# ADicksonLab/AGDIFF

Hardware: AMD Instinct MI355X
Metric: conformers/sec (whole node), GEOM-Drugs 5000-step sampling (higher is better)
Workload: dtype f16x3

## Files before the change

### agdiff_amd/csrc/common.hpp

```cpp
#pragma once
#include <hip/hip_runtime.h>
#include <stdint.h>
#include "agdiff_hip.h"

typedef float f32x4 __attribute__((ext_vector_type(4)));
typedef __bf16 bf16x8 __attribute__((ext_vector_type(8)));
typedef _Float16 f16x8 __attribute__((ext_vector_type(8)));
typedef unsigned int u32x4 __attribute__((ext_vector_type(4)));
typedef __attribute__((address_space(3))) u32x4 lds_u32x4;

#define AG_WAVE 64
#define AG_WG 256
#define AG_TW AGDIFF_TILE

__device__ __forceinline__ int ag_lane() { return threadIdx.x & 63; }
__device__ __forceinline__ int ag_wave_in_wg() { return threadIdx.x >> 6; }

__device__ __forceinline__ f32x4 ag_ld4(const float* __restrict__ p) { return *reinterpret_cast<const f32x4*>(p); }
__device__ __forceinline__ void ag_st4(float* __restrict__ p, f32x4 v) { *reinterpret_cast<f32x4*>(p) = v; }

__device__ __forceinline__ float ag_exp2(float x) { return __builtin_amdgcn_exp2f(x); }
__device__ __forceinline__ float ag_log2(float x) { return __builtin_amdgcn_logf(x); }
__device__ __forceinline__ float ag_rcp(float x) { return __builtin_amdgcn_rcpf(x); }

// ... 238 lines not shown
  } else {
    using V = decltype(x.hi);
    const V wv = __builtin_bit_cast(V, w[part == 2 ? 1 : 0]);
    const V xv = (part == 1) ? x.lo : x.hi;
    o = FLIP ? ag_mfma16(xv, wv, o) : ag_mfma16(wv, xv, o);
  }
}

template <int MODE, bool FLIP>
__device__ __forceinline__ void ag_block_mma_mixed(f32x4& o, const AgIn<MODE>& x, const u32x4 (&w)[2]) {
  static_assert(MODE != AG_F32, "split modes only");
  using V = decltype(x.hi);
  const V wv = __builtin_bit_cast(V, w[1]);
  o = FLIP ? ag_mfma16(x.lo, wv, o) : ag_mfma16(wv, x.lo, o);
}

template <int MODE, bool FLIP>
__device__ __forceinline__ f32x4 ag_block_mma_first(const AgIn<MODE>& x, const u32x4 (&w)[2]) {
  const f32x4 zero = {0.f, 0.f, 0.f, 0.f};
  if constexpr (MODE == AG_F32) {
    const f32x4 wf = __builtin_bit_cast(f32x4, w[0]);
    return FLIP ? __builtin_amdgcn_mfma_f32_16x16x4f32(x.v[0][0], wf[0], zero, 0, 0, 0)
                : __builtin_amdgcn_mfma_f32_16x16x4f32(wf[0], x.v[0][0], zero, 0, 0, 0);
  } else {
    using V = decltype(x.hi);
    const V wv = __builtin_bit_cast(V, w[0]);
    return FLIP ? ag_mfma16(x.hi, wv, zero) : ag_mfma16(wv, x.hi, zero);
  }
}

template <int MODE, bool FLIP, bool KOUTER, int KT, int OT, int X0, int O0, int PF, int NX, int NO>
__device__ __forceinline__ void ag_dense(const AgIn<MODE> (&x)[NX], f32x4 (&o)[NO], const void* wpk, int lane) {
  static_assert(X0 + KT <= NX && O0 + OT <= NO, "tile range");
  constexpr int S = OT * KT;
  constexpr int R = PF + 1;
  u32x4 w[R][2];
  const u32x4* wl = reinterpret_cast<const u32x4*>(wpk) + lane;
#pragma unroll
  for (int s = 0; s < (PF < S ? PF : S); ++s) {
    w[s % R][0] = wl[(s * 2) * 64];
    w[s % R][1] = wl[(s * 2 + 1) * 64];
  }
#pragma unroll
  for (int s = 0; s < S; ++s) {
    const int t = KOUTER ? s / OT : s % KT, ot = KOUTER ? s % OT : s / KT;
    if (s + PF < S) {
      w[(s + PF) % R][0] = wl[((s + PF) * 2) * 64];
      w[(s + PF) % R][1] = wl[((s + PF) * 2 + 1) * 64];
    }
    ag_block_mma<MODE, FLIP>(o[O0 + ot], x[X0 + t], w[s % R]);
    __builtin_amdgcn_sched_barrier(0);
  }
}
template <int MODE, bool FLIP, bool KOUTER, int KT, int OT, int X0, int O0, int NX, int NO>
__device__ __forceinline__ void ag_dense_lds(const AgIn<MODE> (&x)[NX], f32x4 (&o)[NO], const lds_u32x4* wl, int lane) {
  static_assert(X0 + KT <= NX && O0 + OT <= NO, "tile range");
  constexpr int G = (OT % 4 == 0) ? 4 : (OT % 2 == 0) ? 2 : 1;
#pragma unroll
  for (int og = 0; og < OT / G; ++og) {
#pragma unroll
    for (int t = 0; t < KT; ++t) {
      u32x4 w[G][2];
#pragma unroll
      for (int g = 0; g < G; ++g) {
        const int ot = og * G + g;
        const int s = KOUTER ? t * OT + ot : ot * KT + t;
        w[g][0] = wl[(s * 2) * 64 + lane];
        w[g][1] = wl[(s * 2 + 1) * 64 + lane];
      }
#pragma unroll
      for (int part = 0; part < AgParts<MODE>::n; ++part) {
#pragma unroll
        for (int g = 0; g < G; ++g) ag_block_mma_part<MODE, FLIP>(o[O0 + og * G + g], x[X0 + t], w[g], part);
      }
    }
  }
}
template <int MODE, bool FLIP, bool KOUTER, int KT, int OT, int X0, int O0, int PF, int NX, int NO>
__device__ __forceinline__ void ag_dense_split(const AgIn<MODE> (&x)[NX], f32x4 (&o)[NO], const lds_u32x4* w0,
                                               const void* wpk, int lane, int lds_lane) {
  static_assert(X0 + KT <= NX && O0 + OT <= NO, "tile range");
  constexpr int S = OT * KT;
  constexpr int R = PF + 1;
  u32x4 w1[R];
  const u32x4* wl = reinterpret_cast<const u32x4*>(wpk) + 64 + lane;
#pragma unroll
  for (int s = 0; s < (PF < S ? PF : S); ++s) w1[s % R] = wl[(s * 2) * 64];
#pragma unroll
  for (int s = 0; s < S; ++s) {
    const int t = KOUTER ? s / OT : s % KT, ot = KOUTER ? s % OT : s / KT;
    if (s + PF < S) w1[(s + PF) % R] = wl[((s + PF) * 2) * 64];
    u32x4 w[2];
    w[0] = w0[s * 64 + lds_lane];
    w[1] = w1[s % R];
    ag_block_mma<MODE, FLIP>(o[O0 + ot], x[X0 + t], w);
    __builtin_amdgcn_sched_barrier(0);
  }
}
template <int MODE> struct AgPF { static constexpr int v = (MODE == AG_F32) ? 2 : 4; };
__device__ __forceinline__ const void* ag_wblock(const float* wpk, int b) { return wpk + (size_t)b * 512; }


__device__ __forceinline__ int64_t ag_attr_unit(int64_t tile, int t, int u, int lane) {
  return ((tile * 4 + t) * 2 + u) * 64 + (lane & 15) * 4 + (lane >> 4);
}
__device__ __forceinline__ void ag_store_attr(const AgIn<AG_F32>& x, float* frag, int64_t tile, int t, int lane) {
  u32x4* p = reinterpret_cast<u32x4*>(frag);
  p[ag_attr_unit(tile, t, 0, lane)] = __builtin_bit_cast(u32x4, x.v[0]);
  p[ag_attr_unit(tile, t, 1, lane)] = __builtin_bit_cast(u32x4, x.v[1]);
}
__device__ __forceinline__ void ag_store_attr(const AgIn<AG_BF3>& x, float* frag, int64_t tile, int t, int lane) {
  u32x4* p = reinterpret_cast<u32x4*>(frag);
  p[ag_attr_unit(tile, t, 0, lane)] = __builtin_bit_cast(u32x4, x.hi);
  p[ag_attr_unit(tile, t, 1, lane)] = __builtin_bit_cast(u32x4, x.lo);
}
__device__ __forceinline__ void ag_store_attr(const AgIn<AG_H3>& x, float* frag, int64_t tile, int t, int lane) {
  u32x4* p = reinterpret_cast<u32x4*>(frag);
  p[ag_attr_unit(tile, t, 0, lane)] = __builtin_bit_cast(u32x4, x.hi);
  p[ag_attr_unit(tile, t, 1, lane)] = __builtin_bit_cast(u32x4, x.lo);
}
__device__ __forceinline__ void ag_load_attr(AgIn<AG_H3>& x, const float* frag, int64_t tile, int t, int lane) {
  const u32x4* p = reinterpret_cast<const u32x4*>(frag);
  x.hi = __builtin_bit_cast(f16x8, p[ag_attr_unit(tile, t, 0, lane)]);
  x.lo = __builtin_bit_cast(f16x8, p[ag_attr_unit(tile, t, 1, lane)]);
}
__device__ __forceinline__ void ag_load_attr(AgIn<AG_F32>& x, const float* frag, int64_t tile, int t, int lane) {
  const u32x4* p = reinterpret_cast<const u32x4*>(frag);
  x.v[0] = __builtin_bit_cast(f32x4, p[ag_attr_unit(tile, t, 0, lane)]);
// ... 181 lines not shown
```

### agdiff_amd/csrc/edge.hip

```cpp
#include "common.hpp"

namespace {

__device__ __forceinline__ const lds_u32x4* ag_lds_base(const lds_u32x4* p, int lane) {
  const lds_u32x4* b = p + lane;
  asm volatile("" : "+v"(b));
  return b;
}

struct EncArgs {
  const float* fe_w;
  const float* fe_b;
  const float* t1;
  const float* w1_pk;
  const float* t3;
  const float* w23_pk;
  const float* w4_pk;
  const float* b4;
  const int32_t* n_dev;
  const float* e_len;
  const int32_t* e_type;
  float* out_frag;
  float* out_rows;
  const int32_t* row_index;
// ... 33 lines not shown
      for (int t = 0; t < 4; ++t) ag_store_attr(x[t], out_frag, tile, t, lane);
    } else {
#pragma unroll
      for (int t = 0; t < 4; ++t) {
        if (o.p >= 0) ag_store_attr(x[t], out_frag, o.p >> 4, t, q * 16 + (int)(o.p & 15));
        if (o.pm >= 0) ag_store_attr(x[t], out_frag, o.pm >> 4, t, q * 16 + (int)(o.pm & 15));
      }
    }
  }
}

#define AG_PERSIST_WAVES 16
template <int MODE>
__global__ void __launch_bounds__(64 * AG_PERSIST_WAVES, 4) k_edge_encoder(EncArgs a) {
  extern __shared__ u32x4 ag_enc_smem[];
  lds_u32x4* lw1 = (lds_u32x4*)ag_enc_smem;
  lds_u32x4* lw23 = lw1 + 32 * 128;
  lds_u32x4* lw4 = lw23 + 32 * 128;
  if (a.tile_flags && a.tile_flags[0] == 0) return;
  {
    const u32x4* g1 = reinterpret_cast<const u32x4*>(a.w1_pk);
    const u32x4* g2 = reinterpret_cast<const u32x4*>(a.w23_pk);
    const u32x4* g4 = reinterpret_cast<const u32x4*>(a.w4_pk);
    ag_copy_lds(lw1, g1, 32 * 128);
    ag_copy_lds(lw23, g2, 32 * 128);
    ag_copy_lds_map(lw4, g4, 32 * 64, [](int i) { return (i >> 6) * 128 + (i & 63); });
  }
  __syncthreads();
  const int lane0 = ag_lane();
  const int E = *a.n_dev;
  const int64_t stride = (int64_t)gridDim.x * AG_PERSIST_WAVES;
  for (int64_t tile = (int64_t)blockIdx.x * AG_PERSIST_WAVES + (threadIdx.x >> 6); tile < a.max_tiles; tile += stride) {
    if (tile * AG_TW >= E) break;
    const int row_mask = a.tile_flags ? a.tile_flags[1 + tile] : 0xFFFF;
    if (row_mask == 0) continue;
    int lane = lane0;
    asm volatile("" : "+v"(lane));
    const int q = lane >> 4;
    const int64_t e = tile * AG_TW + (lane & 15);
    const bool valid = e < E && ((row_mask >> (lane & 15)) & 1);
    const float d = valid ? a.e_len[e] : 0.0f;
    const int ty = valid ? a.e_type[e] : 0;

    f32x4 y[8];
    AgIn<MODE> x[4];
    {
      f32x4 w[8];
      ag_init_vec<8>(w, a.fe_w, q);
      ag_init_vec<8>(y, a.fe_b, q);
      AG_FOR_TILE(y, 8, ag_gelu(fmaf(w[_t][_r], d, v)));
    }
    ag_cvt_tiles<MODE, 4, 0>(y, x);
    ag_init_vec<8>(y, a.t1 + (size_t)ty * 128, q);
    ag_dense_lds<MODE, false, false, 4, 8, 0, 0>(x, y, ag_lds_base(lw1, lane), 0);
    AG_FOR_TILE(y, 8, ag_gelu(v));
    ag_cvt_tiles<MODE, 4, 0>(y, x);
    ag_init_vec<8>(y, a.t3 + (size_t)ty * 128, q);
    ag_dense_lds<MODE, false, false, 4, 8, 0, 0>(x, y, ag_lds_base(lw23, lane), 0);
    AG_FOR_TILE(y, 8, ag_gelu(v));
    ag_cvt_tiles<MODE, 4, 0>(y, x);
    ag_init_vec<8>(y, a.b4, q);
    ag_dense_split<MODE, false, false, 4, 8, 0, 0, 6>(x, y, ag_lds_base(lw4, lane), a.w4_pk, lane, 0);
    ag_emit_edge_attr<MODE>(y, ag_edge_out(a.pos_index, a.mir_index, e, valid), a.out_frag, a.out_rows, a.row_index,
                            a.pos_index != nullptr, tile, lane);
  }
}

struct GaussArgs {
  const float* offset;
  const float* emb;
  const int32_t* n_dev;
  const float* e_len;
  const int32_t* e_type;
  float* out_frag;
  float* out_rows;
  const int32_t* row_index;
  const int32_t* pos_index;
  const int32_t* mir_index;
  int64_t max_tiles;
  float coeff_log2e;
};

template <int MODE>
__global__ void __launch_bounds__(256) k_edge_gaussian(GaussArgs a) {
  const int64_t tile = (int64_t)blockIdx.x * 4 + (threadIdx.x >> 6);
  const int E = *a.n_dev;
  if (tile >= a.max_tiles || tile * AG_TW >= E) return;
  const int lane = ag_lane();
  const int q = lane >> 4;
  const int64_t e = tile * AG_TW + (lane & 15);
  const bool valid = e < E;
  const float d = valid ? a.e_len[e] : 0.0f;
  const int ty = valid ? a.e_type[e] : 0;
  f32x4 y[8];
  ag_load_row<4, 0>(y, a.offset, q);
  AG_FOR_TILE(y, 4, ag_exp2(a.coeff_log2e * ((d - v) * (d - v))));
  ag_load_row<4, 4>(y, a.emb + (size_t)ty * 64, q);
  ag_emit_edge_attr<MODE>(y, ag_edge_out(a.pos_index, a.mir_index, e, valid), a.out_frag, a.out_rows, a.row_index,
                          a.pos_index != nullptr, tile, lane);
}

struct ScaleArgs {
  const float* dw[2 * AGDIFF_MAX_CONVS];
  const int32_t* n_dev;
  const float* e_len;
  const int32_t* pos_index;
  const int32_t* mir_index;
  const int32_t* e_type;
  const int32_t* type_slot;
  float* out;
  int64_t epad;
// ... 358 lines not shown
  int64_t max_tiles;
};

template <int MODE>
__global__ void __launch_bounds__(64 * AG_PERSIST_WAVES, 4) k_pair_head(HeadArgs a) {
  extern __shared__ u32x4 ag_head_smem[];
  lds_u32x4* lw1 = (lds_u32x4*)ag_head_smem;
  lds_u32x4* lw2 = lw1 + 64 * 128;
  {
    const u32x4* g1 = reinterpret_cast<const u32x4*>(a.hp.w1_pk);
    const u32x4* g2 = reinterpret_cast<const u32x4*>(a.hp.w2_pk);
    ag_copy_lds(lw1, g1, 64 * 128);
    ag_copy_lds(lw2, g2, 16 * 128);
  }
  __syncthreads();
  const int lane0 = ag_lane();
  const int E = *a.n_dev;
  const int64_t stride = (int64_t)gridDim.x * AG_PERSIST_WAVES;
  const int64_t wg = (gridDim.x % 8 == 0) ? (int64_t)(blockIdx.x % 8) * (gridDim.x / 8) + blockIdx.x / 8 : (int64_t)blockIdx.x;
  for (int64_t tile = wg * AG_PERSIST_WAVES + (threadIdx.x >> 6); tile < a.max_tiles; tile += stride) {
    if (tile * AG_TW >= E) break;
    int lane = lane0;
    asm volatile("" : "+v"(lane));
    const int q = lane >> 4;
    const int64_t e = tile * AG_TW + (lane & 15);
    const bool valid = e < E;
    const int s = valid ? a.src[e] : 0, t = valid ? a.dst[e] : 0;
    const int64_t pe = a.pos_index ? (valid ? (int64_t)a.pos_index[e] : 0) : e;
    const int64_t pm = (a.pos_index && valid) ? (int64_t)a.mir_index[e] : -1;

    f32x4 y1[8];
    ag_init_vec<8>(y1, a.hp.b1, q);
    {
      const float* hs = a.node_h + (size_t)s * 128;
      const float* ht = a.node_h + (size_t)t * 128;
      AgIn<MODE> sl[2];
      auto load_slice = [&](AgIn<MODE>& dst, int k) {
        if (k < 4) {
          const f32x4 p0 = ag_ld4(hs + 32 * k + 4 * q) * ag_ld4(ht + 32 * k + 4 * q);
          const f32x4 p1 = ag_ld4(hs + 32 * k + 16 + 4 * q) * ag_ld4(ht + 32 * k + 16 + 4 * q);
          ag_cvt(p0, p1, dst);
        } else if (a.attr_frag && a.pos_index) {
          ag_load_attr(dst, a.attr_frag, pe >> 4, k - 4, q * 16 + (int)(pe & 15));
        } else if (a.attr_frag) {
          ag_load_attr(dst, a.attr_frag, tile, k - 4, lane);
        } else {
          const float* ar = a.attr_rows + (size_t)(valid ? e : 0) * 128 + 32 * (k - 4) + 4 * q;
          ag_cvt(ag_ld4(ar), ag_ld4(ar + 16), dst);
        }
      };
      load_slice(sl[0], 0);
      const lds_u32x4* lw1_lo = ag_lds_base(lw1, lane);
      const lds_u32x4* lw1_hi = ag_lds_base(lw1 + 32 * 128, lane);
#pragma unroll
      for (int k = 0; k < 8; ++k) {
        if (k + 1 < 8) load_slice(sl[(k + 1) & 1], k + 1);
        const lds_u32x4* wk = (k < 4) ? lw1_lo + (k * 8) * 128 : lw1_hi + ((k - 4) * 8) * 128;
        if (k & 1) ag_dense_lds<MODE, false, true, 1, 8, 1, 0>(sl, y1, wk, 0);
        else ag_dense_lds<MODE, false, true, 1, 8, 0, 0>(sl, y1, wk, 0);
      }
    }
    ag_head_act<8>(y1, a.hp.act);
    f32x4 y2[4];
    ag_init_vec<4>(y2, a.hp.b2, q);
    {
      AgIn<MODE> y1b[4];
      ag_report_range<MODE>(ag_absmax<MODE, 8>(y1, 0.0f), a.hp.range_rows, s, valid);
      ag_cvt_tiles<MODE, 4, 0>(y1, y1b);
      ag_dense_lds<MODE, false, false, 4, 4, 0, 0>(y1b, y2, ag_lds_base(lw2, lane), 0);
    }
    ag_head_act<4>(y2, a.hp.act);
    const float o = ag_dot_vec<4>(y2, a.hp.w3, q) + a.hp.b3;
    if (valid && q == 0) {
      a.out[pe] = o;
      if (pm >= 0) a.out[pm] = o;
    }
  }
}

struct RadScaleArgs {
  const float* dw[2 * AGDIFF_MAX_CONVS];
  const int32_t* rad_cnt;
  int32_t* rad_src;
  float* rad_len;
  float* out;
  int64_t rpad;
  int32_t n;
  float cutoff;
  int32_t smooth;
};
__global__ void __launch_bounds__(256) k_rad_scales(RadScaleArgs a) {
  __shared__ float seg[2 * AGDIFF_MAX_CONVS * 100];
  for (int i = threadIdx.x; i < a.n * 100; i += blockDim.x) seg[i] = a.dw[i / 100][i % 100];
  __syncthreads();
  const int64_t row = (int64_t)blockIdx.x * blockDim.x + threadIdx.x;
  if (row >= a.rpad) return;
  const int i = (int)(row / AGDIFF_RAD_STRIDE), k = (int)(row - (int64_t)i * AGDIFF_RAD_STRIDE);
  const int cnt = a.rad_cnt[i];
  if (k >= ((cnt + AG_TW - 1) / AG_TW) * AG_TW) return;
  if (k >= cnt) {
    a.rad_src[row] = i;
    a.rad_len[row] = 0.0f;
    for (int c = 0; c < a.n; ++c) a.out[(size_t)c * a.rpad + row] = 0.0f;
    return;
  }
  const float d = a.rad_len[row];
  const float C = cf_envelope(d, a.cutoff, a.smooth);
  for (int c = 0; c < a.n; ++c) a.out[(size_t)c * a.rpad + row] = cf_dist_weight(seg + c * 100, d) * C;
}

__global__ void k_zero_word(int32_t* p) {
  if (threadIdx.x == 0) *p = 0;
}

struct AttrPolyArgs {
  const float* poly_pk;
  const int32_t* type_slot;
  const int32_t* n_dev;
  const float* e_len;
  const int32_t* e_type;
  float* out_rows;
  int32_t* flags;
// ... 96 lines not shown

template <int MODE, int NKT>
__global__ void __launch_bounds__(64 * AG_PERSIST_WAVES, 4) k_pair_head_poly(HeadPolyArgs a) {
  extern __shared__ u32x4 ag_headp_smem[];
  lds_u32x4* lw1 = (lds_u32x4*)ag_headp_smem;
  lds_u32x4* lwp = lw1 + 32 * 128;
  lds_u32x4* lw2 = lwp + 8 * NKT * 128;
  {
    const u32x4* g1 = reinterpret_cast<const u32x4*>(a.hp.w1_pk);
    const u32x4* gp = reinterpret_cast<const u32x4*>(a.hp.attr_poly_pk);
    const u32x4* g2 = reinterpret_cast<const u32x4*>(a.hp.w2_pk);
    ag_copy_lds(lw1, g1, 32 * 128);
    ag_copy_lds(lwp, gp, 8 * NKT * 128);
    ag_copy_lds(lw2, g2, 16 * 128);
  }
  __syncthreads();
  const int lane0 = ag_lane();
  const int E = a.seg_tile_live ? 0 : *a.n_dev;
  const int64_t stride = (int64_t)gridDim.x * AG_PERSIST_WAVES;
  const int64_t wg = (gridDim.x % 8 == 0) ? (int64_t)(blockIdx.x % 8) * (gridDim.x / 8) + blockIdx.x / 8 : (int64_t)blockIdx.x;
  for (int64_t tile = wg * AG_PERSIST_WAVES + (threadIdx.x >> 6); tile < a.max_tiles; tile += stride) {
    int64_t live_end;
    if (a.seg_tile_live) {
      const int live = a.seg_tile_live[tile];
      if (live == 0) continue;
      live_end = tile * AG_TW + live;
    } else {
      live_end = E;
      if (tile * AG_TW >= E) break;
    }
    int lane = lane0;
    asm volatile("" : "+v"(lane));
    const int q = lane >> 4;
    const int64_t e = tile * AG_TW + (lane & 15);
    const bool valid = e < live_end;
    const int s = valid ? a.src[e] : 0, t = valid ? a.dst[e] : 0;
    const float d = valid ? a.len[e] : 0.0f;
    const int64_t pe = a.pos_index ? (valid ? (int64_t)a.pos_index[e] : 0) : e;
    const int64_t pm = (a.pos_index && valid) ? (int64_t)a.mir_index[e] : -1;

    f32x4 y1[8];
    ag_init_vec<8>(y1, a.hp.b1, q);
    {
      const float* hs = a.node_h + (size_t)s * 128;
      const float* ht = a.node_h + (size_t)t * 128;
      AgIn<MODE> sl[2];
      auto load_slice = [&](AgIn<MODE>& dst, int k) {
        const f32x4 p0 = ag_ld4(hs + 32 * k + 4 * q) * ag_ld4(ht + 32 * k + 4 * q);
        const f32x4 p1 = ag_ld4(hs + 32 * k + 16 + 4 * q) * ag_ld4(ht + 32 * k + 16 + 4 * q);
        ag_cvt(p0, p1, dst);
      };
      load_slice(sl[0], 0);
      const lds_u32x4* lw1_l = ag_lds_base(lw1, lane);
#pragma unroll
      for (int k = 0; k < 4; ++k) {
        if (k + 1 < 4) load_slice(sl[(k + 1) & 1], k + 1);
        if (k & 1) ag_dense_lds<MODE, false, true, 1, 8, 1, 0>(sl, y1, lw1_l + (k * 8) * 128, 0);
        else ag_dense_lds<MODE, false, true, 1, 8, 0, 0>(sl, y1, lw1_l + (k * 8) * 128, 0);
      }
      AgIn<MODE> ph[NKT];
      ag_poly_features<MODE, NKT>(d, a.two_over_rc, q, ph);
      ag_dense_lds<MODE, false, true, NKT, 8, 0, 0>(ph, y1, ag_lds_base(lwp, lane), 0);
    }
    ag_head_act<8>(y1, a.hp.act);
    f32x4 y2[4];
    ag_init_vec<4>(y2, a.hp.b2, q);
    {
      AgIn<MODE> y1b[4];
      ag_report_range<MODE>(ag_absmax<MODE, 8>(y1, 0.0f), a.hp.range_rows, s, valid);
      ag_cvt_tiles<MODE, 4, 0>(y1, y1b);
      ag_dense_lds<MODE, false, false, 4, 4, 0, 0>(y1b, y2, ag_lds_base(lw2, lane), 0);
    }
    ag_head_act<4>(y2, a.hp.act);
    const float o = ag_dot_vec<4>(y2, a.hp.w3, q) + a.hp.b3;
    if (valid && q == 0) {
      a.out[pe] = o;
      if (pm >= 0) a.out[pm] = o;
    }
  }
}

template <int F>
__global__ void __launch_bounds__(AG_WG) k_cfconv_aggregate(const float* __restrict__ x, const float* __restrict__ W,
                                                            const int32_t* __restrict__ in_ptr,
                                                            const int32_t* __restrict__ src, int64_t n,
                                                            float* __restrict__ out) {
  constexpr int LPE = F / 4;
  constexpr int EPI = 64 / LPE;
  const int lane = ag_lane();
  const int64_t node = (int64_t)blockIdx.x * 4 + ag_wave_in_wg();
  if (node >= n) return;
  const int lo = in_ptr[node], hi = in_ptr[node + 1];
  const int sub = lane / LPE, fl = (lane % LPE) * 4;
  f32x4 acc = {0.f, 0.f, 0.f, 0.f};
  for (int e = lo + sub; e < hi; e += EPI) {
    const f32x4 w = ag_ld4(W + (size_t)e * F + fl);
    const f32x4 xv = ag_ld4(x + (size_t)src[e] * F + fl);
    acc += w * xv;
  }
#pragma unroll
  for (int o = LPE; o < 64; o <<= 1) {
#pragma unroll
    for (int q = 0; q < 4; ++q) acc[q] += __shfl_xor(acc[q], o);
  }
  if (sub == 0) ag_st4(out + (size_t)node * F + fl, acc);
}

}

static thread_local const int32_t* g_enc_tile_flags = nullptr;

extern "C" int agdiff_edge_encoder(const agdiff_params_t* p, const int32_t* n_edges_dev, int64_t max_tiles,
                                   const float* e_len, const int32_t* e_type, float* attr_frag, float* attr_rows,
                                   const int32_t* row_index, const int32_t* pos_index, const int32_t* mir_index,
                                   void* stream) {
  if (!p || !n_edges_dev || !e_len || !e_type || (!attr_frag && !attr_rows) || max_tiles < 0 || (!pos_index != !mir_index))
    return AGDIFF_ERR_ARG;
  if (max_tiles == 0) return AGDIFF_OK;
  if (p->edge_encoder == 1) {
    if (!p->ge_offset || !p->ge_emb) return AGDIFF_ERR_ARG;
    GaussArgs g{p->ge_offset, p->ge_emb, n_edges_dev, e_len, e_type, attr_frag, attr_rows, row_index, pos_index, mir_index,
                max_tiles, p->ge_coeff * 1.44269504088896340736f};
    const dim3 grid((unsigned)((max_tiles + 3) / 4));
    ag_by_mode(p->precision, [&](auto M) { k_edge_gaussian<decltype(M)::value><<<grid, dim3(256), 0, (hipStream_t)stream>>>(g); });
// ... 332 lines not shown
```

### agdiff_amd/csrc/node.hip

```cpp
#include "common.hpp"
#include <cstdlib>

namespace {

struct NodeStageArgs {
  agdiff_conv_params_t prev;
  agdiff_conv_params_t next;
  const float* emb;
  const int32_t* atom_type;
  const int32_t* in_ptr;
  const float* agg;
  const float* agg_first;
  float* h;
  const float* h_in;
  float* xs;
  int64_t n;
  int32_t finish;
  int32_t prep;
  int32_t chunk_edges;
  const int32_t* in_ptr2;
  const float* agg2;
  const float* agg_first2;
  int32_t chunk_edges2;
  int32_t* range_rows;
};

struct AggSrc {
  const float* row;
  const float* first;
  int c_lo, c_hi;
  bool has;
};
__device__ __forceinline__ AggSrc ag_agg_src(const int32_t* in_ptr, const float* agg, const float* agg_first, int chunk_e,
                                             int64_t nd) {
  AggSrc r;
  if (!in_ptr) {
    r.has = true;
    r.c_lo = r.c_hi = 0;
    r.row = agg + (size_t)nd * 192;
    r.first = agg_first;
    return r;
  }
  const int lo = in_ptr[nd], hi = in_ptr[nd + 1];
  r.has = hi > lo;
  r.c_lo = lo / chunk_e;
  r.c_hi = r.has ? (hi - 1) / chunk_e : r.c_lo;
  r.row = agg + (size_t)nd * 192;
  r.first = agg_first;
  return r;
}
__device__ __forceinline__ void ag_agg_slice(const AggSrc& r, int k, int q, f32x4& v0, f32x4& v1) {
  v0 = r.has ? ag_ld4(r.row + 32 * k + 4 * q) : f32x4{0.f, 0.f, 0.f, 0.f};
  v1 = r.has ? ag_ld4(r.row + 32 * k + 16 + 4 * q) : f32x4{0.f, 0.f, 0.f, 0.f};
  for (int c = r.c_lo + 1; c <= r.c_hi; ++c) {
    const float* fr = r.first + (size_t)c * 192;
    v0 += ag_ld4(fr + 32 * k + 4 * q);
    v1 += ag_ld4(fr + 32 * k + 16 + 4 * q);
  }
}

#define AG_NODE_LDS_BLOCKS 80
#define AG_NODE_DENSE(KOUTER, KT, OT, X0, O0, x, o, gsrc, lblock)                                   \
  do {                                                                                              \
    if constexpr (LDSW) ag_dense_lds<MODE, false, KOUTER, KT, OT, X0, O0>(x, o, L + (lblock) * 128, lane); \
    else ag_dense<MODE, false, KOUTER, KT, OT, X0, O0, PF>(x, o, gsrc, lane);                       \
  } while (0)
template <int MODE, bool LDSW>
__global__ void __launch_bounds__(LDSW ? 1024 : 256, LDSW ? 1 : 2) k_schnet_node_stage(NodeStageArgs a) {
  extern __shared__ u32x4 ag_node_smem[];
  lds_u32x4* L = (lds_u32x4*)ag_node_smem;
  constexpr int PF = (MODE == AG_F32) ? 3 : 10;
  auto stage_in = [&](int dst_block, const float* src, int nblocks) {
    if constexpr (LDSW) {
      const u32x4* g = reinterpret_cast<const u32x4*>(src);
      ag_copy_lds<4>(L + dst_block * 128, g, nblocks * 128);
    }
  };
  auto sync = [&]() {
    if constexpr (LDSW) __syncthreads();
  };
  const int lane = ag_lane(), q = lane >> 4;
  const int64_t tile = (int64_t)blockIdx.x * (blockDim.x >> 6) + (threadIdx.x >> 6);
  const bool active = tile * AG_TW < a.n;
  const int64_t node = tile * AG_TW + (lane & 15);
  const bool valid = active && node < a.n;
  const int64_t nd = valid ? node : 0;

  f32x4 hv[8];
  if (!a.finish) {
    if (a.prep) stage_in(12, a.next.lin1_pk, 48);
    if (active) ag_load_row<8, 0>(hv, a.emb + (size_t)a.atom_type[nd] * 128, q);
    sync();
  } else {
    stage_in(0, a.prev.lin2a_pk, 32);
    stage_in(32, a.prev.lin2b_pk, 16);
    stage_in(48, a.prev.lin_pk, 32);
    sync();
    f32x4 xc[8];
    AgIn<MODE> ub[8];
    if (active) {
      f32x4 u[16];
      {
        const AggSrc src1 = ag_agg_src(a.in_ptr, a.agg, a.agg_first, a.chunk_edges, nd);
        const bool two = a.in_ptr2 != nullptr;
        const AggSrc src2 = two ? ag_agg_src(a.in_ptr2, a.agg2, a.agg_first2, a.chunk_edges2, nd) : src1;
        ag_init_vec<16>(u, a.prev.lin2_b, q);
        AgIn<MODE> g[2];
        auto load_slice = [&](AgIn<MODE>& dst, int k) {
          f32x4 v0, v1;
          ag_agg_slice(src1, k, q, v0, v1);
          if (two) {
            f32x4 w0, w1;
            ag_agg_slice(src2, k, q, w0, w1);
            v0 += w0;
            v1 += w1;
          }
          ag_cvt(v0, v1, dst);
        };
        load_slice(g[0], 0);
#pragma unroll
        for (int k = 0; k < 6; ++k) {
          if (k + 1 < 6) load_slice(g[(k + 1) & 1], k + 1);
          if (k < 4) {
            if (k & 1) AG_NODE_DENSE(true, 1, 8, 1, 0, g, u, ag_wblock(a.prev.lin2a_pk, k * 8), k * 8);
            else AG_NODE_DENSE(true, 1, 8, 0, 0, g, u, ag_wblock(a.prev.lin2a_pk, k * 8), k * 8);
          } else {
            if (k & 1) AG_NODE_DENSE(true, 1, 8, 1, 8, g, u, ag_wblock(a.prev.lin2b_pk, (k - 4) * 8), 32 + (k - 4) * 8);
            else AG_NODE_DENSE(true, 1, 8, 0, 8, g, u, ag_wblock(a.prev.lin2b_pk, (k - 4) * 8), 32 + (k - 4) * 8);
          }
        }
      }
      AG_FOR_TILE(u, 16, ag_ssp_base2(v));
      ag_report_range<MODE>(ag_absmax<MODE, 16>(u, 0.0f), a.range_rows, nd, valid);
      ag_cvt_tiles<MODE, 8, 0>(u, ub);
      ag_init_vec<8>(xc, a.prev.lin_b, q);
      AG_NODE_DENSE(false, 8, 4, 0, 0, ub, xc, a.prev.lin_pk, 48);
    }
    sync();
    stage_in(0, a.prev.lin_pk + (size_t)32 * 512, 32);
    stage_in(32, a.prev.gate1_pk, 16);
    sync();
    if (active) {
      AG_NODE_DENSE(false, 8, 4, 0, 4, ub, xc, ag_wblock(a.prev.lin_pk, 32), 0);
      f32x4 g1[4];
      ag_init_vec<4>(g1, a.prev.gate1_b, q);
      {
        AgIn<MODE> xb[4];
        ag_report_range<MODE>(ag_absmax<MODE, 8>(xc, 0.0f), a.range_rows, nd, valid);
        ag_cvt_tiles<MODE, 4, 0>(xc, xb);
        AG_NODE_DENSE(false, 4, 4, 0, 0, xb, g1, a.prev.gate1_pk, 32);
      }
      AG_FOR_TILE(g1, 4, ag_relu(v));
      const float gate = ag_sigmoid(ag_dot_vec<4>(g1, a.prev.gate2_w, q) + a.prev.gate2_b);
      AG_FOR_TILE(xc, 8, v * gate);
    }
    sync();
    stage_in(0, a.prev.scale1_pk, 4);
    stage_in(4, a.prev.scale2_pk, 8);
    if (a.prep) stage_in(12, a.next.lin1_pk, 48);
    sync();
    if (active) {
      f32x4 s1[2] = {{0.f, 0.f, 0.f, 0.f}, {0.f, 0.f, 0.f, 0.f}};
      f32x4 s2[8];
      {
        AgIn<MODE> xb[4];
        ag_cvt_tiles<MODE, 4, 0>(xc, xb);
        AG_NODE_DENSE(false, 4, 1, 0, 0, xb, s1, a.prev.scale1_pk, 0);
      }
      AG_FOR_TILE(s1, 1, ag_relu(v));
#pragma unroll
      for (int t = 0; t < 8; ++t) s2[t] = f32x4{0.f, 0.f, 0.f, 0.f};
      {
        AgIn<MODE> sb[1];
        ag_report_range<MODE>(ag_absmax<MODE, 2>(s1, 0.0f), a.range_rows, nd, valid);
        ag_cvt_tiles<MODE, 1, 0>(s1, sb);
        AG_NODE_DENSE(false, 1, 8, 0, 0, sb, s2, a.prev.scale2_pk, 4);
      }
      ag_load_row<8, 0>(hv, a.h_in + (size_t)nd * 128, q);
#pragma unroll
      for (int t = 0; t < 8; ++t)
#pragma unroll
        for (int r = 0; r < 4; ++r) hv[t][r] = hv[t][r] + xc[t][r] * ag_sigmoid(s2[t][r]);
    }
  }
  if (!active) return;
  ag_report_range<MODE>(ag_absmax<MODE, 8>(hv, 0.0f), a.range_rows, nd, valid, 255.0f);
  if (valid) ag_store_row<8, 0>(hv, a.h + (size_t)node * 128, q);
  if (a.prep) {
    f32x4 xo[12];
    ag_init_vec<12>(xo, a.next.lin1_b, q);
    {
      AgIn<MODE> hb[4];
      ag_cvt_tiles<MODE, 4, 0>(hv, hb);
      AG_NODE_DENSE(false, 4, 12, 0, 0, hb, xo, a.next.lin1_pk, 12);
    }
    AG_FOR_TILE(xo, 12, ag_lrelu(v));
    ag_report_range<MODE>(ag_absmax<MODE, 12>(xo, 0.0f), a.range_rows, nd, valid, 60000.0f);
    if (valid) ag_store_row<12, 0>(xo, a.xs + (size_t)node * 192, q);
  }
}

template <int MODE>
__device__ __forceinline__ void ag_xch_put(lds_u32x4* x, int kt, const AgIn<MODE>& v, int lane) {
  if constexpr (MODE == AG_F32) {
    x[(kt * 2) * 64 + lane] = __builtin_bit_cast(u32x4, v.v[0]);
    x[(kt * 2 + 1) * 64 + lane] = __builtin_bit_cast(u32x4, v.v[1]);
  } else {
    x[(kt * 2) * 64 + lane] = __builtin_bit_cast(u32x4, v.hi);
    x[(kt * 2 + 1) * 64 + lane] = __builtin_bit_cast(u32x4, v.lo);
  }
}
template <int MODE>
__device__ __forceinline__ void ag_xch_get(const lds_u32x4* x, int kt, AgIn<MODE>& v, int lane) {
  if constexpr (MODE == AG_F32) {
    v.v[0] = __builtin_bit_cast(f32x4, x[(kt * 2) * 64 + lane]);
    v.v[1] = __builtin_bit_cast(f32x4, x[(kt * 2 + 1) * 64 + lane]);
  } else {
    v.hi = __builtin_bit_cast(decltype(v.hi), x[(kt * 2) * 64 + lane]);
    v.lo = __builtin_bit_cast(decltype(v.lo), x[(kt * 2 + 1) * 64 + lane]);
  }
}

template <int MODE, bool FINISH, bool PREP>
__global__ void __launch_bounds__(256, 2) k_schnet_node_stage_split(NodeStageArgs a) {
  __shared__ u32x4 ag_split_xch[20 * 128];
  __shared__ float ag_split_red[4][16];
  lds_u32x4* xch = (lds_u32x4*)ag_split_xch;
  const int lane = ag_lane(), q = lane >> 4;
  const int w = __builtin_amdgcn_readfirstlane(ag_wave_in_wg());
  const int64_t tile = blockIdx.x;
  const int64_t node = tile * AG_TW + (lane & 15);
  const bool valid = node < a.n;
  const int64_t nd = valid ? node : 0;
  constexpr int NF = FINISH ? 38 : 0, NS = NF + (PREP ? 12 : 0);
  constexpr int PF = 12, R = PF + 1;

  auto block_of = [&](int s) -> const float* {
    if (FINISH && s < 8) return a.prev.lin2a_pk + (size_t)((s >> 1) * 8 + 2 * w + (s & 1)) * 512;
    if (FINISH && s < 12) return a.prev.lin2b_pk + (size_t)(((s - 8) >> 1) * 8 + 2 * w + (s & 1)) * 512;
    if (FINISH && s < 28) return a.prev.lin_pk + (size_t)((2 * w + ((s - 12) >> 3)) * 8 + ((s - 12) & 7)) * 512;
    if (FINISH && s < 32) return a.prev.gate1_pk + (size_t)(w * 4 + (s - 28)) * 512;
    if (FINISH && s < 36) return a.prev.scale1_pk + (size_t)(s - 32) * 512;
    if (FINISH && s < 38) return a.prev.scale2_pk + (size_t)(2 * w + (s - 36)) * 512;
    return a.next.lin1_pk + (size_t)((3 * w + ((s - NF) >> 2)) * 4 + ((s - NF) & 3)) * 512;
  };
  u32x4 ring[R][2];
  auto request = [&](int s) {
// ... 182 lines not shown
      bool on[U];
#pragma unroll
      for (int u = 0; u < U; ++u) {
        const int s = __shfl(my_src, 32 * half + ((k + u) & 31)), r = __shfl(my_row, 32 * half + ((k + u) & 31));
        on[u] = s >= 0;
        hv[u] = ag_ld4(hbase + (size_t)(on[u] ? s : 0) * 128 + 4 * j);
        ev[u] = ag_ld4(a.l_attr_rows + (size_t)r * 128 + 4 * j);
      }
#pragma unroll
      for (int u = 0; u < U; ++u) {
#pragma unroll
        for (int r = 0; r < 4; ++r) acc[r] += on[u] ? ag_relu(hv[u][r] + ev[u][r]) : 0.0f;
      }
    }
  }
  acc = acc + a.gp.one_plus_eps * hself;
  if (valid) *reinterpret_cast<f32x4*>(a.h_out + (size_t)node * 128 + 4 * j) = acc;
}

template <int MODE, bool LDSW>
__global__ void __launch_bounds__(LDSW ? 1024 : 256, LDSW ? 1 : 2) k_gin_layer(GinArgs a) {
  extern __shared__ u32x4 ag_gin_smem[];
  lds_u32x4* L = (lds_u32x4*)ag_gin_smem;
  constexpr int PF = (MODE == AG_F32) ? 3 : 10;
  if constexpr (LDSW) {
    const u32x4* g1 = reinterpret_cast<const u32x4*>(a.gp.w1_pk);
    const u32x4* g2 = reinterpret_cast<const u32x4*>(a.gp.w2_pk);
    ag_copy_lds(L, g1, 32 * 128);
    ag_copy_lds(L + 32 * 128, g2, 32 * 128);
  }
  const int lane = ag_lane(), q = lane >> 4;
  const int64_t tile = (int64_t)blockIdx.x * (blockDim.x >> 6) + (threadIdx.x >> 6);
  const bool active = tile * AG_TW < a.n;
  const int64_t node = tile * AG_TW + (lane & 15);
  const bool valid = active && node < a.n;
  const int64_t nd = valid ? node : 0;
  const float* hin_self = a.emb ? a.emb + (size_t)a.atom_type[nd] * 128 : a.h_in + (size_t)nd * 128;

  f32x4 m[8];
#pragma unroll
  for (int t = 0; t < 8; ++t) m[t] = f32x4{0.f, 0.f, 0.f, 0.f};
  f32x4 hself[8];
  if (active) {
    ag_load_row<8, 0>(m, a.h_out + (size_t)nd * 128, q);
    ag_load_row<8, 0>(hself, hin_self, q);
  }
  if constexpr (LDSW) __syncthreads();
  if (!active) return;
  f32x4 y1[8];
  ag_init_vec<8>(y1, a.gp.b1, q);
  {
    AgIn<MODE> mb[4];
    ag_cvt_tiles<MODE, 4, 0>(m, mb);
    AG_NODE_DENSE(false, 4, 8, 0, 0, mb, y1, a.gp.w1_pk, 0);
  }
  AG_FOR_TILE(y1, 8, ag_relu(v));
  ag_init_vec<8>(m, a.gp.b2, q);
  {
    AgIn<MODE> yb[4];
    ag_report_range<MODE>(ag_absmax<MODE, 8>(y1, 0.0f), a.range_rows, nd, valid);
    ag_cvt_tiles<MODE, 4, 0>(y1, yb);
    AG_NODE_DENSE(false, 4, 8, 0, 0, yb, m, a.gp.w2_pk, 32);
  }
  if (a.gp.relu_out) { AG_FOR_TILE(m, 8, ag_relu(v)); }
#pragma unroll
  for (int t = 0; t < 8; ++t) m[t] += hself[t];
  ag_report_range<MODE>(ag_absmax<MODE, 8>(m, 0.0f), a.range_rows, nd, valid, 255.0f);
  if (valid) ag_store_row<8, 0>(m, a.h_out + (size_t)node * 128, q);
}

template <int MODE>
__global__ void __launch_bounds__(1024, 1) k_gin_layer_persistent(GinArgs a) {
  constexpr bool LDSW = true;
  extern __shared__ u32x4 ag_gin_smem[];
  lds_u32x4* L = (lds_u32x4*)ag_gin_smem;
  constexpr int PF = (MODE == AG_F32) ? 3 : 10;
  if constexpr (LDSW) {
    const u32x4* g1 = reinterpret_cast<const u32x4*>(a.gp.w1_pk);
    const u32x4* g2 = reinterpret_cast<const u32x4*>(a.gp.w2_pk);
    ag_copy_lds(L, g1, 32 * 128);
    ag_copy_lds(L + 32 * 128, g2, 32 * 128);
    __syncthreads();
  }
  const int lane = ag_lane(), q = lane >> 4;
  const int64_t tiles = (a.n + AG_TW - 1) / AG_TW;
  const int64_t stride = (int64_t)gridDim.x * (blockDim.x >> 6);
  for (int64_t tile = (int64_t)blockIdx.x * (blockDim.x >> 6) + (threadIdx.x >> 6); tile < tiles; tile += stride) {
    const int64_t node = tile * AG_TW + (lane & 15);
    const bool valid = node < a.n;
    const int64_t nd = valid ? node : 0;
    const float* hin_self = a.emb ? a.emb + (size_t)a.atom_type[nd] * 128 : a.h_in + (size_t)nd * 128;
    f32x4 m[8], hself[8];
    ag_load_row<8, 0>(m, a.h_out + (size_t)nd * 128, q);
    ag_load_row<8, 0>(hself, hin_self, q);
    f32x4 y1[8];
    ag_init_vec<8>(y1, a.gp.b1, q);
    {
      AgIn<MODE> mb[4];
      ag_cvt_tiles<MODE, 4, 0>(m, mb);
      AG_NODE_DENSE(false, 4, 8, 0, 0, mb, y1, a.gp.w1_pk, 0);
    }
    AG_FOR_TILE(y1, 8, ag_relu(v));
    ag_init_vec<8>(m, a.gp.b2, q);
    {
      AgIn<MODE> yb[4];
      ag_report_range<MODE>(ag_absmax<MODE, 8>(y1, 0.0f), a.range_rows, nd, valid);
      ag_cvt_tiles<MODE, 4, 0>(y1, yb);
      AG_NODE_DENSE(false, 4, 8, 0, 0, yb, m, a.gp.w2_pk, 32);
    }
    if (a.gp.relu_out) { AG_FOR_TILE(m, 8, ag_relu(v)); }
#pragma unroll
    for (int t = 0; t < 8; ++t) m[t] += hself[t];
    ag_report_range<MODE>(ag_absmax<MODE, 8>(m, 0.0f), a.range_rows, nd, valid, 255.0f);
    if (valid) ag_store_row<8, 0>(m, a.h_out + (size_t)node * 128, q);
  }
}

struct UpdateArgs {
  agdiff_step_args_t s;
  const int32_t* graph_ptr;
  const int32_t* loc_src;
  const int32_t* loc_dst;
  const int32_t* loc_out_ptr;
  const int32_t* loc_in_ptr;
  const int32_t* loc_in_eid;
  const float* l_len;
  const float* l_inv;
  const int32_t* in_ptr;
  const int32_t* out_ptr;
  const int32_t* ref2dst;
  const int32_t* e_src;
  const int32_t* e_dst;
  const int32_t* e_type;
  const float* e_len;
  const float* e_inv;
  int32_t* nan_flag;
  int32_t parts;
};

__device__ __forceinline__ void clip3(float& x, float& y, float& z, float limit) {
  const float nrm = sqrtf(x * x + y * y + z * z);
  if (nrm > limit) {
    const float d = limit / nrm;
    x *= d; y *= d; z *= d;
  }
}

__global__ void __launch_bounds__(1024) k_langevin_update(UpdateArgs a) {
  const int g = blockIdx.x;
  const int g0 = a.graph_ptr[g], n = a.graph_ptr[g + 1] - g0;
  __shared__ float red[3][16];
  __shared__ int nanw[16];
  float sx = 0.f, sy = 0.f, sz = 0.f;
  int bad = 0;
  const int was_bad = a.nan_flag[1 + g];
  const int P = a.parts, part = threadIdx.x & (P - 1);
  const int per_pass = blockDim.x / P;
  for (int base = 0; base < n; base += per_pass) {
    const int li = base + (int)(threadIdx.x / P);
    const bool on = li < n;
    const int i = g0 + (on ? li : 0);
// ... 603 lines not shown
```

Measured before the change: 172.1.

## Double-buffer LDS weight reads across MFMA blocks with chained ring prefetch

Adds a two-slot register ring for LDS weight fragments. The next block's weights are read from LDS while the current block's MFMAs issue, and sched_barrier masks keep DS reads and MFMAs interleaved. Chained calls across k-slices prefetch the first block of the next slice, or of the poly-feature weights, so there is no LDS latency bubble at slice boundaries. The change is applied to the edge head MLPs and the non-persistent GIN layer. It costs extra VGPRs for the ring, which may reduce occupancy.

Result: no change. 172.9 (median of 6 runs) (+0.5%).

```diff
diff --git a/agdiff_amd/csrc/common.hpp b/agdiff_amd/csrc/common.hpp
--- a/agdiff_amd/csrc/common.hpp
+++ b/agdiff_amd/csrc/common.hpp
@@ -314,28 +314,73 @@
     __builtin_amdgcn_sched_barrier(0);
   }
 }
-template <int MODE, bool FLIP, bool KOUTER, int KT, int OT, int X0, int O0, int NX, int NO>
+#define AG_SCHED_KEEP_DS_MFMA 0x476
+template <int H> struct AgLdsRing { u32x4 w[2][H][2]; };
+template <int MODE, bool FLIP, bool KOUTER, int KT, int OT, int X0, int O0, int H, int NX, int NO>
+__device__ __forceinline__ void ag_dense_lds_ring(const AgIn<MODE> (&x)[NX], f32x4 (&o)[NO], const lds_u32x4* wl, int lane,
+                                                  AgLdsRing<H>& r, bool primed, const lds_u32x4* wl_next, int next_stride) {
+  static_assert(X0 + KT <= NX && O0 + OT <= NO && H >= 1 && OT % H == 0, "tile range");
+  constexpr int NS = (OT / H) * KT;
+  auto read = [&](int n) {
+    const int oh = n / KT, t = n % KT;
+#pragma unroll
+    for (int g = 0; g < H; ++g) {
+      const int ot = oh * H + g;
+      const int s = KOUTER ? t * OT + ot : ot * KT + t;
+      r.w[n & 1][g][0] = wl[(s * 2) * 64 + lane];
+      r.w[n & 1][g][1] = wl[(s * 2 + 1) * 64 + lane];
+    }
+  };
+  if (!primed) read(0);
+#pragma unroll
+  for (int n = 0; n < NS; ++n) {
+    if (n + 1 < NS) {
+      read(n + 1);
+    } else if (wl_next) {
+      static_assert(NS % 2 == 0, "a chained call ends in slot 1");
+#pragma unroll
+      for (int g = 0; g < H; ++g) {
+        r.w[0][g][0] = wl_next[(g * next_stride * 2) * 64 + lane];
+        r.w[0][g][1] = wl_next[(g * next_stride * 2 + 1) * 64 + lane];
+      }
+    }
+    __builtin_amdgcn_sched_barrier(AG_SCHED_KEEP_DS_MFMA);
+    const int oh = n / KT, t = n % KT;
+#pragma unroll
+    for (int part = 0; part < AgParts<MODE>::n; ++part) {
+#pragma unroll
+      for (int g = 0; g < H; ++g) ag_block_mma_part<MODE, FLIP>(o[O0 + oh * H + g], x[X0 + t], r.w[n & 1][g], part);
+    }
+    __builtin_amdgcn_sched_barrier(AG_SCHED_KEEP_DS_MFMA);
+  }
+}
+template <int MODE, bool FLIP, bool KOUTER, int KT, int OT, int X0, int O0, int H, int NX, int NO>
 __device__ __forceinline__ void ag_dense_lds(const AgIn<MODE> (&x)[NX], f32x4 (&o)[NO], const lds_u32x4* wl, int lane) {
   static_assert(X0 + KT <= NX && O0 + OT <= NO, "tile range");
-  constexpr int G = (OT % 4 == 0) ? 4 : (OT % 2 == 0) ? 2 : 1;
-#pragma unroll
-  for (int og = 0; og < OT / G; ++og) {
-#pragma unroll
-    for (int t = 0; t < KT; ++t) {
-      u32x4 w[G][2];
-#pragma unroll
-      for (int g = 0; g < G; ++g) {
-        const int ot = og * G + g;
-        const int s = KOUTER ? t * OT + ot : ot * KT + t;
-        w[g][0] = wl[(s * 2) * 64 + lane];
-        w[g][1] = wl[(s * 2 + 1) * 64 + lane];
+  if constexpr (H == 0) {
+    constexpr int G = (OT % 4 == 0) ? 4 : (OT % 2 == 0) ? 2 : 1;
+#pragma unroll
+    for (int og = 0; og < OT / G; ++og) {
+#pragma unroll
+      for (int t = 0; t < KT; ++t) {
+        u32x4 w[G][2];
+#pragma unroll
+        for (int g = 0; g < G; ++g) {
+          const int ot = og * G + g;
+          const int s = KOUTER ? t * OT + ot : ot * KT + t;
+          w[g][0] = wl[(s * 2) * 64 + lane];
+          w[g][1] = wl[(s * 2 + 1) * 64 + lane];
+        }
+#pragma unroll
+        for (int part = 0; part < AgParts<MODE>::n; ++part) {
+#pragma unroll
+          for (int g = 0; g < G; ++g) ag_block_mma_part<MODE, FLIP>(o[O0 + og * G + g], x[X0 + t], w[g], part);
+        }
       }
-#pragma unroll
-      for (int part = 0; part < AgParts<MODE>::n; ++part) {
-#pragma unroll
-        for (int g = 0; g < G; ++g) ag_block_mma_part<MODE, FLIP>(o[O0 + og * G + g], x[X0 + t], w[g], part);
-      }
-    }
+    }
+  } else {
+    AgLdsRing<H> r;
+    ag_dense_lds_ring<MODE, FLIP, KOUTER, KT, OT, X0, O0, H>(x, o, wl, lane, r, false, nullptr, 0);
   }
 }
 template <int MODE, bool FLIP, bool KOUTER, int KT, int OT, int X0, int O0, int PF, int NX, int NO>
diff --git a/agdiff_amd/csrc/edge.hip b/agdiff_amd/csrc/edge.hip
--- a/agdiff_amd/csrc/edge.hip
+++ b/agdiff_amd/csrc/edge.hip
@@ -109,11 +109,11 @@
     }
     ag_cvt_tiles<MODE, 4, 0>(y, x);
     ag_init_vec<8>(y, a.t1 + (size_t)ty * 128, q);
-    ag_dense_lds<MODE, false, false, 4, 8, 0, 0>(x, y, ag_lds_base(lw1, lane), 0);
+    ag_dense_lds<MODE, false, false, 4, 8, 0, 0, 0>(x, y, ag_lds_base(lw1, lane), 0);
     AG_FOR_TILE(y, 8, ag_gelu(v));
     ag_cvt_tiles<MODE, 4, 0>(y, x);
     ag_init_vec<8>(y, a.t3 + (size_t)ty * 128, q);
-    ag_dense_lds<MODE, false, false, 4, 8, 0, 0>(x, y, ag_lds_base(lw23, lane), 0);
+    ag_dense_lds<MODE, false, false, 4, 8, 0, 0, 0>(x, y, ag_lds_base(lw23, lane), 0);
     AG_FOR_TILE(y, 8, ag_gelu(v));
     ag_cvt_tiles<MODE, 4, 0>(y, x);
     ag_init_vec<8>(y, a.b4, q);
@@ -578,12 +578,14 @@
       load_slice(sl[0], 0);
       const lds_u32x4* lw1_lo = ag_lds_base(lw1, lane);
       const lds_u32x4* lw1_hi = ag_lds_base(lw1 + 32 * 128, lane);
+      auto wslice = [&](int k) { return (k < 4) ? lw1_lo + (k * 8) * 128 : lw1_hi + ((k - 4) * 8) * 128; };
+      AgLdsRing<2> ring;
 #pragma unroll
       for (int k = 0; k < 8; ++k) {
         if (k + 1 < 8) load_slice(sl[(k + 1) & 1], k + 1);
-        const lds_u32x4* wk = (k < 4) ? lw1_lo + (k * 8) * 128 : lw1_hi + ((k - 4) * 8) * 128;
-        if (k & 1) ag_dense_lds<MODE, false, true, 1, 8, 1, 0>(sl, y1, wk, 0);
-        else ag_dense_lds<MODE, false, true, 1, 8, 0, 0>(sl, y1, wk, 0);
+        const lds_u32x4* wn = (k + 1 < 8) ? wslice(k + 1) : nullptr;
+        if (k & 1) ag_dense_lds_ring<MODE, false, true, 1, 8, 1, 0, 2>(sl, y1, wslice(k), 0, ring, k > 0, wn, 1);
+        else ag_dense_lds_ring<MODE, false, true, 1, 8, 0, 0, 2>(sl, y1, wslice(k), 0, ring, k > 0, wn, 1);
       }
     }
     ag_head_act<8>(y1, a.hp.act);
@@ -593,7 +595,7 @@
       AgIn<MODE> y1b[4];
       ag_report_range<MODE>(ag_absmax<MODE, 8>(y1, 0.0f), a.hp.range_rows, s, valid);
       ag_cvt_tiles<MODE, 4, 0>(y1, y1b);
-      ag_dense_lds<MODE, false, false, 4, 4, 0, 0>(y1b, y2, ag_lds_base(lw2, lane), 0);
+      ag_dense_lds<MODE, false, false, 4, 4, 0, 0, 2>(y1b, y2, ag_lds_base(lw2, lane), 0);
     }
     ag_head_act<4>(y2, a.hp.act);
     const float o = ag_dot_vec<4>(y2, a.hp.w3, q) + a.hp.b3;
@@ -796,15 +798,18 @@
       };
       load_slice(sl[0], 0);
       const lds_u32x4* lw1_l = ag_lds_base(lw1, lane);
+      const lds_u32x4* lwp_l = ag_lds_base(lwp, lane);
+      AgLdsRing<2> ring;
 #pragma unroll
       for (int k = 0; k < 4; ++k) {
         if (k + 1 < 4) load_slice(sl[(k + 1) & 1], k + 1);
-        if (k & 1) ag_dense_lds<MODE, false, true, 1, 8, 1, 0>(sl, y1, lw1_l + (k * 8) * 128, 0);
-        else ag_dense_lds<MODE, false, true, 1, 8, 0, 0>(sl, y1, lw1_l + (k * 8) * 128, 0);
+        const lds_u32x4* wn = (k + 1 < 4) ? lw1_l + ((k + 1) * 8) * 128 : lwp_l;
+        if (k & 1) ag_dense_lds_ring<MODE, false, true, 1, 8, 1, 0, 2>(sl, y1, lw1_l + (k * 8) * 128, 0, ring, k > 0, wn, 1);
+        else ag_dense_lds_ring<MODE, false, true, 1, 8, 0, 0, 2>(sl, y1, lw1_l + (k * 8) * 128, 0, ring, k > 0, wn, 1);
       }
       AgIn<MODE> ph[NKT];
       ag_poly_features<MODE, NKT>(d, a.two_over_rc, q, ph);
-      ag_dense_lds<MODE, false, true, NKT, 8, 0, 0>(ph, y1, ag_lds_base(lwp, lane), 0);
+      ag_dense_lds_ring<MODE, false, true, NKT, 8, 0, 0, 2>(ph, y1, lwp_l, 0, ring, true, nullptr, 0);
     }
     ag_head_act<8>(y1, a.hp.act);
     f32x4 y2[4];
@@ -813,7 +818,7 @@
       AgIn<MODE> y1b[4];
       ag_report_range<MODE>(ag_absmax<MODE, 8>(y1, 0.0f), a.hp.range_rows, s, valid);
       ag_cvt_tiles<MODE, 4, 0>(y1, y1b);
-      ag_dense_lds<MODE, false, false, 4, 4, 0, 0>(y1b, y2, ag_lds_base(lw2, lane), 0);
+      ag_dense_lds<MODE, false, false, 4, 4, 0, 0, 2>(y1b, y2, ag_lds_base(lw2, lane), 0);
     }
     ag_head_act<4>(y2, a.hp.act);
     const float o = ag_dot_vec<4>(y2, a.hp.w3, q) + a.hp.b3;
diff --git a/agdiff_amd/csrc/node.hip b/agdiff_amd/csrc/node.hip
--- a/agdiff_amd/csrc/node.hip
+++ b/agdiff_amd/csrc/node.hip
@@ -60,9 +60,9 @@
 }
 
 #define AG_NODE_LDS_BLOCKS 80
-#define AG_NODE_DENSE(KOUTER, KT, OT, X0, O0, x, o, gsrc, lblock)                                   \
+#define AG_NODE_DENSE(H, KOUTER, KT, OT, X0, O0, x, o, gsrc, lblock)                                \
   do {                                                                                              \
-    if constexpr (LDSW) ag_dense_lds<MODE, false, KOUTER, KT, OT, X0, O0>(x, o, L + (lblock) * 128, lane); \
+    if constexpr (LDSW) ag_dense_lds<MODE, false, KOUTER, KT, OT, X0, O0, H>(x, o, L + (lblock) * 128, lane); \
     else ag_dense<MODE, false, KOUTER, KT, OT, X0, O0, PF>(x, o, gsrc, lane);                       \
   } while (0)
 template <int MODE, bool LDSW>
@@ -122,11 +122,11 @@
         for (int k = 0; k < 6; ++k) {
           if (k + 1 < 6) load_slice(g[(k + 1) & 1], k + 1);
           if (k < 4) {
-            if (k & 1) AG_NODE_DENSE(true, 1, 8, 1, 0, g, u, ag_wblock(a.prev.lin2a_pk, k * 8), k * 8);
-            else AG_NODE_DENSE(true, 1, 8, 0, 0, g, u, ag_wblock(a.prev.lin2a_pk, k * 8), k * 8);
+            if (k & 1) AG_NODE_DENSE(0, true, 1, 8, 1, 0, g, u, ag_wblock(a.prev.lin2a_pk, k * 8), k * 8);
+            else AG_NODE_DENSE(0, true, 1, 8, 0, 0, g, u, ag_wblock(a.prev.lin2a_pk, k * 8), k * 8);
           } else {
-            if (k & 1) AG_NODE_DENSE(true, 1, 8, 1, 8, g, u, ag_wblock(a.prev.lin2b_pk, (k - 4) * 8), 32 + (k - 4) * 8);
-            else AG_NODE_DENSE(true, 1, 8, 0, 8, g, u, ag_wblock(a.prev.lin2b_pk, (k - 4) * 8), 32 + (k - 4) * 8);
+            if (k & 1) AG_NODE_DENSE(0, true, 1, 8, 1, 8, g, u, ag_wblock(a.prev.lin2b_pk, (k - 4) * 8), 32 + (k - 4) * 8);
+            else AG_NODE_DENSE(0, true, 1, 8, 0, 8, g, u, ag_wblock(a.prev.lin2b_pk, (k - 4) * 8), 32 + (k - 4) * 8);
           }
         }
       }
@@ -134,21 +134,21 @@
       ag_report_range<MODE>(ag_absmax<MODE, 16>(u, 0.0f), a.range_rows, nd, valid);
       ag_cvt_tiles<MODE, 8, 0>(u, ub);
       ag_init_vec<8>(xc, a.prev.lin_b, q);
-      AG_NODE_DENSE(false, 8, 4, 0, 0, ub, xc, a.prev.lin_pk, 48);
+      AG_NODE_DENSE(0, false, 8, 4, 0, 0, ub, xc, a.prev.lin_pk, 48);
     }
     sync();
     stage_in(0, a.prev.lin_pk + (size_t)32 * 512, 32);
     stage_in(32, a.prev.gate1_pk, 16);
     sync();
     if (active) {
-      AG_NODE_DENSE(false, 8, 4, 0, 4, ub, xc, ag_wblock(a.prev.lin_pk, 32), 0);
+      AG_NODE_DENSE(0, false, 8, 4, 0, 4, ub, xc, ag_wblock(a.prev.lin_pk, 32), 0);
       f32x4 g1[4];
       ag_init_vec<4>(g1, a.prev.gate1_b, q);
       {
         AgIn<MODE> xb[4];
         ag_report_range<MODE>(ag_absmax<MODE, 8>(xc, 0.0f), a.range_rows, nd, valid);
         ag_cvt_tiles<MODE, 4, 0>(xc, xb);
-        AG_NODE_DENSE(false, 4, 4, 0, 0, xb, g1, a.prev.gate1_pk, 32);
+        AG_NODE_DENSE(0, false, 4, 4, 0, 0, xb, g1, a.prev.gate1_pk, 32);
       }
       AG_FOR_TILE(g1, 4, ag_relu(v));
       const float gate = ag_sigmoid(ag_dot_vec<4>(g1, a.prev.gate2_w, q) + a.prev.gate2_b);
@@ -165,7 +165,7 @@
       {
         AgIn<MODE> xb[4];
         ag_cvt_tiles<MODE, 4, 0>(xc, xb);
-        AG_NODE_DENSE(false, 4, 1, 0, 0, xb, s1, a.prev.scale1_pk, 0);
+        AG_NODE_DENSE(0, false, 4, 1, 0, 0, xb, s1, a.prev.scale1_pk, 0);
       }
       AG_FOR_TILE(s1, 1, ag_relu(v));
 #pragma unroll
@@ -174,7 +174,7 @@
         AgIn<MODE> sb[1];
         ag_report_range<MODE>(ag_absmax<MODE, 2>(s1, 0.0f), a.range_rows, nd, valid);
         ag_cvt_tiles<MODE, 1, 0>(s1, sb);
-        AG_NODE_DENSE(false, 1, 8, 0, 0, sb, s2, a.prev.scale2_pk, 4);
+        AG_NODE_DENSE(0, false, 1, 8, 0, 0, sb, s2, a.prev.scale2_pk, 4);
       }
       ag_load_row<8, 0>(hv, a.h_in + (size_t)nd * 128, q);
 #pragma unroll
@@ -192,7 +192,7 @@
     {
       AgIn<MODE> hb[4];
       ag_cvt_tiles<MODE, 4, 0>(hv, hb);
-      AG_NODE_DENSE(false, 4, 12, 0, 0, hb, xo, a.next.lin1_pk, 12);
+      AG_NODE_DENSE(0, false, 4, 12, 0, 0, hb, xo, a.next.lin1_pk, 12);
     }
     AG_FOR_TILE(xo, 12, ag_lrelu(v));
     ag_report_range<MODE>(ag_absmax<MODE, 12>(xo, 0.0f), a.range_rows, nd, valid, 60000.0f);
@@ -481,7 +481,7 @@
   {
     AgIn<MODE> mb[4];
     ag_cvt_tiles<MODE, 4, 0>(m, mb);
-    AG_NODE_DENSE(false, 4, 8, 0, 0, mb, y1, a.gp.w1_pk, 0);
+    AG_NODE_DENSE(1, false, 4, 8, 0, 0, mb, y1, a.gp.w1_pk, 0);
   }
   AG_FOR_TILE(y1, 8, ag_relu(v));
   ag_init_vec<8>(m, a.gp.b2, q);
@@ -489,7 +489,7 @@
     AgIn<MODE> yb[4];
     ag_report_range<MODE>(ag_absmax<MODE, 8>(y1, 0.0f), a.range_rows, nd, valid);
     ag_cvt_tiles<MODE, 4, 0>(y1, yb);
-    AG_NODE_DENSE(false, 4, 8, 0, 0, yb, m, a.gp.w2_pk, 32);
+    AG_NODE_DENSE(1, false, 4, 8, 0, 0, yb, m, a.gp.w2_pk, 32);
   }
   if (a.gp.relu_out) { AG_FOR_TILE(m, 8, ag_relu(v)); }
 #pragma unroll
@@ -527,7 +527,7 @@
     {
       AgIn<MODE> mb[4];
       ag_cvt_tiles<MODE, 4, 0>(m, mb);
-      AG_NODE_DENSE(false, 4, 8, 0, 0, mb, y1, a.gp.w1_pk, 0);
+      AG_NODE_DENSE(0, false, 4, 8, 0, 0, mb, y1, a.gp.w1_pk, 0);
     }
     AG_FOR_TILE(y1, 8, ag_relu(v));
     ag_init_vec<8>(m, a.gp.b2, q);
@@ -535,7 +535,7 @@
       AgIn<MODE> yb[4];
       ag_report_range<MODE>(ag_absmax<MODE, 8>(y1, 0.0f), a.range_rows, nd, valid);
       ag_cvt_tiles<MODE, 4, 0>(y1, yb);
-      AG_NODE_DENSE(false, 4, 8, 0, 0, yb, m, a.gp.w2_pk, 32);
+      AG_NODE_DENSE(0, false, 4, 8, 0, 0, yb, m, a.gp.w2_pk, 32);
     }
     if (a.gp.relu_out) { AG_FOR_TILE(m, 8, ag_relu(v)); }
 #pragma unroll
```
